# bupt-ai-cz/HIAST

Hardware: AMD Instinct MI355X
Metric: self-training images/sec (fwd+bwd+pseudo-label) at 1024x512 (higher is better)
Workload: dtype fp16

## Files before the change

### hiast_amd/csrc/conv_launch.h

```cpp
#pragma once
#include <stdlib.h>

#include "common.h"

namespace hiast {

struct IGeo {
    int H, W, Ho, Wo, stride, dil;
};

}

struct ConvLaunch {
    const void* x = nullptr;
    const void* wp = nullptr;
    void* y = nullptr;
    const void* res = nullptr;
    const void* res_gate = nullptr;
    int gate_mask = 0;
    const float* gamma = nullptr;
    const float* beta = nullptr;
    const float* mean = nullptr;
    const float* var = nullptr;
    float eps = 0.0f;
    int relu = 0;
    int64_t M = 0;
    int K = 0, N = 0, taps = 1;
    hiast::IGeo geo = {0, 0, 0, 0, 1, 1};
    int fmt = HIAST_FMT_BF16;
    int out_f32 = 0;
    float* stats = nullptr;
    int stats_rows = 0;
    int stats_mode = 0;
    hipStream_t st = nullptr;

    int planes() const { return hiast_fmt_planes(fmt); }
    bool f16() const { return fmt == HIAST_FMT_FP16; }
};

enum class ConvFamily { XCONV, XCONV2, TILE_F16, TILE };

struct ConvRoute {
    ConvFamily family = ConvFamily::TILE;
    int BN = 0, BM = 0;
    bool half9 = false;
    int rows = 0;
};

static inline int conv_panel_streams(int64_t M, int NG, int panel_rows)
{
    static const int env_cus = [] { const char* e = getenv("HIAST_XCONV_CUS"); const int v = e ? atoi(e) : 0; return v >= 8 && v <= 256 ? v : 0; }();
    const long long npanel = (M + panel_rows - 1) / panel_rows;
    long long streams = (env_cus ? env_cus : hiast_grid_cus()) / NG / 8 * 8;
    if (streams < 8) streams = 8;
    if (streams > npanel) streams = (npanel + 7) / 8 * 8;
    return (int)streams;
}

ConvRoute ig_route(const ConvLaunch& c);
int hiast_igemm_launch(const ConvLaunch& c);
int hiast_igemm_launch_f16(const ConvLaunch& c, const ConvRoute& r);
int hiast_xconv_ok(const ConvLaunch& c);
int hiast_xconv_stats_rows(int64_t M, int N);
int hiast_xconv_launch(const ConvLaunch& c, const ConvRoute& r);
int hiast_xconv2_ok(const ConvLaunch& c);
int hiast_xconv2_launch(const ConvLaunch& c);
int hiast_gemm_nt_launch(const float* x, const float* w, float* y, int64_t M, int K, int N, hipStream_t st);
```

### hiast_amd/csrc/igemm.hip

```cpp
#include "igemm_kernel.h"

namespace hiast {

template <int PL>
__device__ __forceinline__ size_t ig_wp_elem(int n, int t, int k, int taps, int KO)
{
    const size_t row = ((size_t)n * taps + t) * PL * KO;
    return PL == 2 ? row + (size_t)(k >> 5) * 64 + (k & 31) : row + k;
}

template <int PL, bool F16 = false>
__global__ __launch_bounds__(256) void pack_conv_weight_kernel(const float* __restrict__ w,
                                                               unsigned short* __restrict__ wp,
                                                               unsigned short* __restrict__ wpt, int N, int K, int taps,
                                                               int mode)
{
    const long long idx = (long long)blockIdx.x * 256 + threadIdx.x;
    if (idx >= (long long)N * taps * K) return;
    const int k = (int)(idx % K);
    const int t = (int)((idx / K) % taps);
    const int n = (int)(idx / ((long long)K * taps));
    const float v = w[((size_t)n * K + k) * taps + t];
    unsigned short h, l = 0;
    if (F16) h = H16<true>::enc(v);
    else ig_split(v, h, l);
    if (mode != 1) {
        unsigned short* d = wp + ig_wp_elem<PL>(n, t, k, taps, K);
        d[0] = h;
        if (PL == 2) d[32] = l;
    }
    if (mode != 0) {
        unsigned short* d = (mode == 1 ? wp : wpt) + ig_wp_elem<PL>(k, taps - 1 - t, n, taps, N);
        d[0] = h;
        if (PL == 2) d[32] = l;
    }
}

constexpr int PK_PITCH = 72;

template <int PL, bool F16 = false>
__device__ __forceinline__ void pack_tile(const float* __restrict__ w, unsigned short* __restrict__ wp,
                                          unsigned short* __restrict__ wpt, int N, int K, int taps, int mode, int n0,
                                          int k0, unsigned short* lds)
{
    constexpr int TN = PL == 1 ? 32 : 16;
    unsigned short* hi = lds;
    unsigned short* lo = lds + (PL == 2 ? TN * taps * PK_PITCH : 0);
    unsigned short* fwd = (mode == 1) ? nullptr : wp;
    unsigned short* adj = (mode == 0) ? nullptr : (mode == 1 ? wp : wpt);
    const int run = 64 * taps;
    for (int nh = 0; nh < 64; nh += TN) {
        if (nh) __syncthreads();
        for (int e = threadIdx.x; e < TN * run; e += 256) {
            const int n = e / run, r = e - n * run;
            const int k = r / taps, t = r - k * taps;
            const float v = w[((size_t)(n0 + nh + n) * K + k0) * taps + r];
            unsigned short h, l = 0;
            if (F16) h = H16<true>::enc(v);
            else ig_split(v, h, l);
            hi[(n * taps + t) * PK_PITCH + k] = h;
            if (PL == 2) lo[(n * taps + t) * PK_PITCH + k] = l;
        }
        __syncthreads();
        if (fwd) {
            for (int e = threadIdx.x; e < TN * taps * 8; e += 256) {
                const int c = e & 7, nt = e >> 3;
                const int n = nt / taps, t = nt - n * taps;
                const uint4 vh = *reinterpret_cast<const uint4*>(&hi[nt * PK_PITCH + c * 8]);
                unsigned short* d = fwd + ig_wp_elem<PL>(n0 + nh + n, t, k0 + c * 8, taps, K);
                *reinterpret_cast<uint4*>(d) = vh;
                if (PL == 2) *reinterpret_cast<uint4*>(d + 32) = *reinterpret_cast<const uint4*>(&lo[nt * PK_PITCH + c * 8]);
            }
        }
        if (adj) {
            for (int e = threadIdx.x; e < 64 * taps * (TN / 8); e += 256) {
                const int c = e % (TN / 8), kt = e / (TN / 8);
                const int k = kt / taps, t = kt - k * taps;
                unsigned short vh[8], vl[8];
#pragma unroll
                for (int j = 0; j < 8; ++j) {
                    vh[j] = hi[((c * 8 + j) * taps + t) * PK_PITCH + k];
                    if (PL == 2) vl[j] = lo[((c * 8 + j) * taps + t) * PK_PITCH + k];
                }
                unsigned short* d = adj + ig_wp_elem<PL>(k0 + k, taps - 1 - t, n0 + nh + c * 8, taps, N);
                *reinterpret_cast<uint4*>(d) = make_uint4(vh[0] | (unsigned)vh[1] << 16, vh[2] | (unsigned)vh[3] << 16,
                                                          vh[4] | (unsigned)vh[5] << 16, vh[6] | (unsigned)vh[7] << 16);
                if (PL == 2)
                    *reinterpret_cast<uint4*>(d + 32) = make_uint4(vl[0] | (unsigned)vl[1] << 16, vl[2] | (unsigned)vl[3] << 16,
                                                                   vl[4] | (unsigned)vl[5] << 16, vl[6] | (unsigned)vl[7] << 16);
            }
        }
    }
}

template <int PL, bool F16 = false>
__global__ __launch_bounds__(256) void pack_conv_weight_tiled_kernel(const float* __restrict__ w,
                                                                     unsigned short* __restrict__ wp,
                                                                     unsigned short* __restrict__ wpt, int N, int K,
                                                                     int taps, int mode)
{
    extern __shared__ __attribute__((aligned(16))) unsigned short lds[];
    const int kt = K / 64;
    pack_tile<PL, F16>(w, wp, wpt, N, K, taps, mode, (int)(blockIdx.x / kt) * 64, (int)(blockIdx.x % kt) * 64, lds);
}

__global__ __launch_bounds__(256) void pack_conv_weight_multi_kernel(const hiast_pack_rec* __restrict__ table,
                                                                     const int32_t* __restrict__ chunk_tensor,
                                                                     const int64_t* __restrict__ chunk_start)
{
    extern __shared__ __attribute__((aligned(16))) unsigned short lds[];
    const hiast_pack_rec r = table[chunk_tensor[blockIdx.x]];
    const int kt = r.K / 64;
    const int tile = (int)chunk_start[blockIdx.x];
    const int n0 = (tile / kt) * 64, k0 = (tile % kt) * 64;
    if (r.planes == HIAST_FMT_SPLIT_BF16)
        pack_tile<2>(r.w, (unsigned short*)r.wp, (unsigned short*)r.wpt, r.N, r.K, r.taps, r.mode, n0, k0, lds);
    else if (r.planes == HIAST_FMT_FP16)
        pack_tile<1, true>(r.w, (unsigned short*)r.wp, (unsigned short*)r.wpt, r.N, r.K, r.taps, r.mode, n0, k0, lds);
    else
        pack_tile<1>(r.w, (unsigned short*)r.wp, (unsigned short*)r.wpt, r.N, r.K, r.taps, r.mode, n0, k0, lds);
}

__global__ __launch_bounds__(256) void to_planes_kernel(const float* __restrict__ x, unsigned short* __restrict__ p,
                                                        long long M, int C)
{
    const long long total8 = M * C / 8;
    for (long long i = (long long)blockIdx.x * 256 + threadIdx.x; i < total8; i += (long long)gridDim.x * 256) {
        const long long m = (i * 8) / C;
        const int c = (int)((i * 8) - m * C);
        const float4 a = reinterpret_cast<const float4*>(x)[2 * i], b = reinterpret_cast<const float4*>(x)[2 * i + 1];
        const float v[8] = {a.x, a.y, a.z, a.w, b.x, b.y, b.z, b.w};
        unsigned ph[4], pl_[4];
#pragma unroll
        for (int q = 0; q < 4; ++q) {
            unsigned short h0, l0, h1, l1;
            ig_split(v[2 * q], h0, l0);
            ig_split(v[2 * q + 1], h1, l1);
            ph[q] = (unsigned)h0 | ((unsigned)h1 << 16);
            pl_[q] = (unsigned)l0 | ((unsigned)l1 << 16);
        }
        unsigned short* dst = p + ig_elem<2>((size_t)m, c, C);
        *reinterpret_cast<uint4*>(dst) = make_uint4(ph[0], ph[1], ph[2], ph[3]);
        *reinterpret_cast<uint4*>(dst + 32) = make_uint4(pl_[0], pl_[1], pl_[2], pl_[3]);
    }
}

__global__ __launch_bounds__(256) void from_planes_kernel(const unsigned short* __restrict__ p, float* __restrict__ x,
                                                          long long M, int C)
{
    const long long total8 = M * C / 8;
    for (long long i = (long long)blockIdx.x * 256 + threadIdx.x; i < total8; i += (long long)gridDim.x * 256) {
        const long long m = (i * 8) / C;
        const int c = (int)((i * 8) - m * C);
        const unsigned short* src = p + ig_elem<2>((size_t)m, c, C);
        const uint4 h = *reinterpret_cast<const uint4*>(src), l = *reinterpret_cast<const uint4*>(src + 32);
        const unsigned wh[4] = {h.x, h.y, h.z, h.w}, wl[4] = {l.x, l.y, l.z, l.w};
        float v[8];
#pragma unroll
        for (int q = 0; q < 4; ++q) {
            v[2 * q] = __uint_as_float(wh[q] << 16) + __uint_as_float(wl[q] << 16);
            v[2 * q + 1] = __uint_as_float(wh[q] & 0xFFFF0000u) + __uint_as_float(wl[q] & 0xFFFF0000u);
        }
        reinterpret_cast<float4*>(x)[2 * i] = make_float4(v[0], v[1], v[2], v[3]);
        reinterpret_cast<float4*>(x)[2 * i + 1] = make_float4(v[4], v[5], v[6], v[7]);
    }
}

}

struct IgEnv {
    int half;
    int bn;
    int ragged_off;
    int cosched0;
};
static const IgEnv& ig_env()
{
    static const IgEnv env = [] {
        IgEnv e;
        const char* v = getenv("HIAST_IGEMM_HALF");
        e.half = v ? (atoi(v) != 0) : -1;
        v = getenv("HIAST_IGEMM_BN");
        const int bn = v ? atoi(v) : 0;
        e.bn = (bn == 64 || bn == 128 || bn == 256) ? bn : 0;
        e.ragged_off = getenv("HIAST_IGEMM_RAGGED") != nullptr;
        v = getenv("HIAST_IGEMM_COSCHED");
        e.cosched0 = v && atoi(v) != 0;
        return e;
    }();
    return env;
}
static thread_local int ig_cosched_tls = -1, ig_half_tls = -1;
extern "C" int hiast_igemm_set_half(int v)
{
    const int prev = ig_half_tls;
    ig_half_tls = v < 0 ? -1 : (v != 0);
    return prev;
}
extern "C" int hiast_igemm_set_cosched(int on)
{
    const int prev = ig_cosched_tls;
    ig_cosched_tls = on < 0 ? -1 : (on != 0);
    return prev;
}
static int ig_half_forced() { return ig_half_tls >= 0 ? ig_half_tls : ig_env().half; }
static int ig_cosched() { return ig_cosched_tls >= 0 ? ig_cosched_tls : ig_env().cosched0; }

#ifndef IG_HALF_AUTO
#define IG_HALF_BLOCKS(M, N) ((((M) + 255) / 256) * (((N) % 256 == 0) ? (N) / 256 : (N) / 128))
#define IG_HALF_AUTO(M, K, N) (IG_HALF_BLOCKS(M, N) <= 64 || (IG_HALF_BLOCKS(M, N) <= 128 && !ig_cosched()))
#endif
static int ig_half_tile(int64_t M, int K, int N, int taps, int out_f32)
{
    if (taps != 1 || out_f32 || N % 128 != 0 || M < 4096) return 0;
    if (ig_half_forced() >= 0) return ig_half_forced();
    return IG_HALF_AUTO(M, K, N);
}
static int ig_half_tile9(int64_t M, int N, int PL, bool bn_relu_only)
{
    if (PL != 2 || !bn_relu_only || N % 128 != 0 || M < 4096) return 0;
    if (ig_half_forced() >= 0) return ig_half_forced();
    return IG_HALF_AUTO(M, 0, N);
}

ConvRoute ig_route(const ConvLaunch& c)
{
    ConvRoute r;
    if (c.stats_mode != 2 && hiast_xconv_ok(c)) {
        r.family = ConvFamily::XCONV;
        r.rows = hiast_xconv_stats_rows(c.M, c.N);
        return r;
    }
    if (c.stats_mode == 0 && !c.f16() && hiast_xconv2_ok(c)) {
        r.family = ConvFamily::XCONV2;
        return r;
    }
    r.family = c.f16() ? ConvFamily::TILE_F16 : ConvFamily::TILE;
    r.BN = (c.N % 256 == 0) ? 256 : ((c.N % 128 == 0) ? 128 : 64);
    const bool plain = !c.mean && !c.gamma && !c.res && !c.relu && !c.res_gate && c.stats_mode == 0;
    if (plain && !c.out_f32 && r.BN == 128 && c.N > 512 && !ig_env().ragged_off) r.BN = 256;
    if (const int v = ig_env().bn) {
        if (c.N % v == 0) r.BN = v;
    }
    r.half9 = c.taps == 9 && !c.out_f32 && c.geo.stride == 1 &&
              ig_half_tile9(c.M, c.N, c.planes(), c.mean && c.relu && !c.res && !c.res_gate && c.stats_mode == 0) != 0;
    const bool half = r.half9 || (c.geo.stride >= 0 && ig_half_tile(c.M, c.K, c.N, c.taps, c.out_f32) != 0);
    if (half) r.BN = 128;
    r.BM = half ? 128 : hiast::IG_BM;
    r.rows = (int)((c.M + r.BM - 1) / r.BM);
    return r;
}

int hiast_igemm_launch(const ConvLaunch& in)
{
    ConvLaunch c = in;
    if (c.stats_mode != 2) c.stats_mode = c.stats ? 1 : 0;
    const int H = c.geo.H, W = c.geo.W, stride = c.geo.stride, dil = c.geo.dil;
    if (!hiast_fmt_ok(c.fmt)) return HIAST_E_RANGE;
    const int planes = c.planes();
    if (c.stats_mode == 2) {
        if (!c.stats || !c.res || !c.mean || !c.var || planes != 1 || c.out_f32 || c.relu || c.res_gate || c.N % 8) return HIAST_E_RANGE;
    } else {
        if (c.stats && (planes != 1 || c.out_f32 || c.res || c.relu)) return HIAST_E_RANGE;
        if ((c.stats || c.res_gate) && c.mean) return HIAST_E_RANGE;
    }
    if (c.res_gate && (planes != 1 || !c.res || c.relu || c.out_f32 || (!c.gate_mask && (((uintptr_t)c.res_gate) & 15)))) return HIAST_E_RANGE;
    if (!c.x || !c.wp || !c.y || (c.mean && !c.var)) return HIAST_E_ARG;
    if (c.M <= 0 || c.K <= 0 || c.N <= 0) return HIAST_E_ARG;
    if ((planes != 1 && planes != 2) || (c.taps != 1 && c.taps != 9)) return HIAST_E_RANGE;
    if ((c.K * planes) % 64 != 0 || c.N % 64 != 0 || c.M > (1ll << 31) - 512) return HIAST_E_RANGE;
    if (c.out_f32 && c.res) return HIAST_E_RANGE;
    if ((((uintptr_t)c.x) | ((uintptr_t)c.wp) | ((uintptr_t)c.y) | ((uintptr_t)c.res)) & 15) return HIAST_E_RANGE;
    c.geo = {0, 0, 0, 0, 1, 1};
    size_t in_pix = (size_t)c.M;
    if (c.taps != 1 && stride == -2) {
        if (H <= 0 || W <= 0 || dil != 1 || planes != 1 || c.out_f32) return HIAST_E_ARG;
        const int Hs = (H - 1) / 2 + 1, Ws = (W - 1) / 2 + 1;
        if (c.M % ((int64_t)H * W) != 0) return HIAST_E_ARG;
        c.geo = {Hs, Ws, H, W, -2, 1};
        in_pix = (size_t)(c.M / ((int64_t)H * W)) * Hs * Ws;
    } else if (c.taps != 1) {
        if (H <= 0 || W <= 0 || stride <= 0 || dil <= 0) return HIAST_E_ARG;
        const int Ho = (H - 1) / stride + 1, Wo = (W - 1) / stride + 1;
        if (c.M % ((int64_t)Ho * Wo) != 0) return HIAST_E_ARG;
        c.geo = {H, W, Ho, Wo, stride, dil};
        in_pix = (size_t)(c.M / ((int64_t)Ho * Wo)) * H * W;
    }
    if (in_pix * planes * c.K * 2 >= (1ull << 31) || (size_t)c.N * c.taps * planes * c.K * 2 >= (1ull << 31)) return HIAST_E_RANGE;
    const ConvRoute r = ig_route(c);
    if (c.stats_mode != 0 && c.stats_rows != r.rows) return HIAST_E_ARG;
    switch (r.family) {
    case ConvFamily::XCONV: return hiast_xconv_launch(c, r);
    case ConvFamily::XCONV2: return hiast_xconv2_launch(c);
    case ConvFamily::TILE_F16: return hiast_igemm_launch_f16(c, r);
    case ConvFamily::TILE: break;
    }
    if (planes == 2) return c.out_f32 ? launch_igemm_t<2, true>(c, r) : launch_igemm_t<2, false>(c, r);
    return c.out_f32 ? launch_igemm_t<1, true>(c, r) : launch_igemm_t<1, false>(c, r);
}

extern "C" int hiast_igemm_dgrad_bn_stats(const void* dy, const void* wpt, void* da, int B, int H, int W, int Cin, int Cout,
                                          int taps, int dil, const void* bn_x, const float* gamma, const float* beta,
                                          const float* save_mean, const float* save_invstd, float* partial, int partial_rows,
                                          int fmt, hiast_stream_t stream)
{
    if (fmt != HIAST_FMT_BF16 && fmt != HIAST_FMT_FP16) return HIAST_E_RANGE;
    if (B <= 0 || H <= 0 || W <= 0) return HIAST_E_ARG;
    if (!bn_x || !save_mean || !save_invstd || !partial) return HIAST_E_ARG;
    if ((((uintptr_t)save_mean) | ((uintptr_t)save_invstd) | ((uintptr_t)gamma) | ((uintptr_t)beta)) & 15) return HIAST_E_RANGE;
    ConvLaunch c;
    c.x = dy; c.wp = wpt; c.y = da; c.res = bn_x;
    c.gamma = gamma; c.beta = beta; c.mean = save_mean; c.var = save_invstd;
    c.M = (int64_t)B * H * W; c.K = Cin; c.N = Cout; c.taps = taps;
    c.geo.H = H; c.geo.W = W; c.geo.dil = dil;
    c.fmt = fmt;
    c.stats = partial; c.stats_rows = partial_rows; c.stats_mode = 2;
    c.st = (hipStream_t)stream;
    return hiast_igemm_launch(c);
}

extern "C" int hiast_igemm_dgrad_s2(const void* dy, const void* wpt, void* dx, int B, int H, int W, int Cin, int Cout, int fmt,
                                    hiast_stream_t stream)
{
    if (fmt != HIAST_FMT_BF16 && fmt != HIAST_FMT_FP16) return HIAST_E_RANGE;
    if (B <= 0 || H <= 0 || W <= 0) return HIAST_E_ARG;
    ConvLaunch c;
    c.x = dy; c.wp = wpt; c.y = dx;
    c.M = (int64_t)B * H * W; c.K = Cout; c.N = Cin; c.taps = 9;
    c.geo.H = H; c.geo.W = W; c.geo.stride = -2;
    c.fmt = fmt;
    c.st = (hipStream_t)stream;
    return hiast_igemm_launch(c);
}

extern "C" int hiast_igemm_bn_act(const void* x, const void* wp, const float* gamma, const float* beta,
                                  const float* mean, const float* var, float eps, const void* res, int relu, void* y,
                                  int B, int H, int W, int Cin, int Cout, int taps, int stride, int dil, int fmt,
                                  int out_f32, float* stats, int stats_rows, const void* res_gate, int gate_mask,
                                  hiast_stream_t stream)
{
    if (B <= 0 || H <= 0 || W <= 0) return HIAST_E_ARG;
    if (taps == 1 && stride != 1) return HIAST_E_RANGE;
    const int Ho = taps == 1 ? H : (H - 1) / stride + 1, Wo = taps == 1 ? W : (W - 1) / stride + 1;
    ConvLaunch c;
    c.x = x; c.wp = wp; c.y = y; c.res = res; c.res_gate = res_gate; c.gate_mask = gate_mask;
    c.gamma = gamma; c.beta = beta; c.mean = mean; c.var = var; c.eps = eps;
    c.relu = relu;
    c.M = (int64_t)B * Ho * Wo; c.K = Cin; c.N = Cout; c.taps = taps;
    c.geo.H = H; c.geo.W = W; c.geo.stride = stride; c.geo.dil = dil;
    c.fmt = fmt; c.out_f32 = out_f32;
    c.stats = stats; c.stats_rows = stats_rows;
    c.st = (hipStream_t)stream;
    return hiast_igemm_launch(c);
}

extern "C" int hiast_igemm_stats_rows(int64_t M, int Cin, int Cout, int taps, int fmt)
{
    if (M <= 0 || Cin <= 0 || Cout <= 0) return 0;
    ConvLaunch c;
    c.M = M; c.K = Cin; c.N = Cout; c.taps = taps; c.fmt = fmt;
    c.stats_mode = 1;
    return ig_route(c).rows;
}
extern "C" int hiast_igemm_dgrad_bn_stats_rows(int64_t M, int Cin, int Cout, int taps)
{
    if (M <= 0) return 0;
    ConvLaunch c;
    c.M = M; c.K = Cin; c.N = Cout; c.taps = taps;
    c.stats_mode = 2;
    return ig_route(c).rows;
}

#ifdef IG_STAMP
namespace hiast {
__global__ void ig_stamp_copy_kernel(unsigned* dst)
{
    for (int i = blockIdx.x * blockDim.x + threadIdx.x; i < 1024 * 8 * 8 + 32 * 64; i += gridDim.x * blockDim.x) dst[i] = ig_stamp_buf[i];
}
}
extern "C" int hiast_igemm_debug_stamps(unsigned* dst_device)
{
    hipLaunchKernelGGL(hiast::ig_stamp_copy_kernel, dim3(64), dim3(256), 0, 0, dst_device);
    return (int)hipDeviceSynchronize();
}
#endif

extern "C" int hiast_pack_conv_weight(const float* w, int N, int K, int taps, int fmt, int transpose, void* wp,
                                      void* wpt, hiast_stream_t stream)
{
    if (!w || !wp) return HIAST_E_ARG;
    if (N <= 0 || K <= 0 || taps <= 0) return HIAST_E_ARG;
    const int planes = fmt;
    if (!hiast_fmt_ok(fmt) || transpose < 0 || transpose > 2) return HIAST_E_RANGE;
    if (transpose == 2 && !wpt) return HIAST_E_ARG;
    if (planes == HIAST_FMT_SPLIT_BF16 && ((transpose != 1 && K % 32 != 0) || (transpose != 0 && N % 32 != 0))) return HIAST_E_RANGE;
    const long long total = (long long)N * K * taps;
    if (N % 64 == 0 && K % 64 == 0 && taps <= 9 && !((((uintptr_t)wp) | ((uintptr_t)wpt)) & 15)) {
        const dim3 tg((unsigned)((N / 64) * (K / 64)));
        const size_t lds_bytes = (size_t)32 * taps * hiast::PK_PITCH * sizeof(unsigned short);
        if (planes == HIAST_FMT_SPLIT_BF16)
            hipLaunchKernelGGL(hiast::pack_conv_weight_tiled_kernel<2>, tg, dim3(256), lds_bytes, (hipStream_t)stream, w,
                               (unsigned short*)wp, (unsigned short*)wpt, N, K, taps, transpose);
        else if (planes == HIAST_FMT_FP16)
            hipLaunchKernelGGL((hiast::pack_conv_weight_tiled_kernel<1, true>), tg, dim3(256), lds_bytes, (hipStream_t)stream, w,
                               (unsigned short*)wp, (unsigned short*)wpt, N, K, taps, transpose);
        else
            hipLaunchKernelGGL(hiast::pack_conv_weight_tiled_kernel<1>, tg, dim3(256), lds_bytes, (hipStream_t)stream, w,
                               (unsigned short*)wp, (unsigned short*)wpt, N, K, taps, transpose);
        HIAST_CHECK_LAUNCH();
        return 0;
    }
    const dim3 grid((unsigned)((total + 255) / 256));
    if (planes == HIAST_FMT_SPLIT_BF16)
        hipLaunchKernelGGL(hiast::pack_conv_weight_kernel<2>, grid, dim3(256), 0, (hipStream_t)stream, w,
                           (unsigned short*)wp, (unsigned short*)wpt, N, K, taps, transpose);
    else if (planes == HIAST_FMT_FP16)
        hipLaunchKernelGGL((hiast::pack_conv_weight_kernel<1, true>), grid, dim3(256), 0, (hipStream_t)stream, w,
                           (unsigned short*)wp, (unsigned short*)wpt, N, K, taps, transpose);
    else
        hipLaunchKernelGGL(hiast::pack_conv_weight_kernel<1>, grid, dim3(256), 0, (hipStream_t)stream, w,
                           (unsigned short*)wp, (unsigned short*)wpt, N, K, taps, transpose);
    HIAST_CHECK_LAUNCH();
    return 0;
}

namespace hiast {

template <int INK, int PL, bool F16 = false>
__global__ __launch_bounds__(256) void stem_tail_kernel(const void* __restrict__ xv, const float* __restrict__ gamma,
                                                        const float* __restrict__ beta, const float* __restrict__ mean,
                                                        const float* __restrict__ var, float eps,
                                                        unsigned short* __restrict__ out, int B, int H, int W, int C, int Ho,
                                                        int Wo)
{
    const int G = C >> 3;
    const long long total = (long long)B * Ho * Wo * G;
    const long long stride = (long long)gridDim.x * 256;
    long long i = (long long)blockIdx.x * 256 + threadIdx.x;
    if (i >= total) return;
    const int cg = (int)(i % G);
    float sc[8], sh[8];
#pragma unroll
    for (int k = 0; k < 8; ++k) {
        const int c = cg * 8 + k;
        const float invstd = 1.0f / sqrtf(var[c] + eps);
        sc[k] = (gamma ? gamma[c] : 1.0f) * invstd;
        sh[k] = fmaf(-mean[c], sc[k], beta ? beta[c] : 0.0f);
    }
    for (; i < total; i += stride) {
        const long long pix = i / G;
        const int xo = (int)(pix % Wo);
        const int yo = (int)((pix / Wo) % Ho);
        const int b = (int)(pix / ((long long)Wo * Ho));
        float m[8];
#pragma unroll
        for (int k = 0; k < 8; ++k) m[k] = -INFINITY;
#pragma unroll
        for (int dy = 0; dy < 3; ++dy) {
            const int yy = 2 * yo - 1 + dy;
            if (yy < 0 || yy >= H) continue;
#pragma unroll
            for (int dx = 0; dx < 3; ++dx) {
                const int xx = 2 * xo - 1 + dx;
                if (xx < 0 || xx >= W) continue;
                const size_t off = (((size_t)b * H + yy) * W + xx) * C + cg * 8;
                float v[8];
                if (INK != 0) {
                    const uint4 r = *reinterpret_cast<const uint4*>(reinterpret_cast<const unsigned short*>(xv) + off);
                    const unsigned w4[4] = {r.x, r.y, r.z, r.w};
#pragma unroll
                    for (int q = 0; q < 4; ++q) {
                        v[2 * q] = H16<INK == 2>::lo(w4[q]);
                        v[2 * q + 1] = H16<INK == 2>::hi(w4[q]);
                    }
                } else {
                    const float4 a = *reinterpret_cast<const float4*>(reinterpret_cast<const float*>(xv) + off);
                    const float4 c4 = *reinterpret_cast<const float4*>(reinterpret_cast<const float*>(xv) + off + 4);
                    v[0] = a.x; v[1] = a.y; v[2] = a.z; v[3] = a.w; v[4] = c4.x; v[5] = c4.y; v[6] = c4.z; v[7] = c4.w;
                }
#pragma unroll
                for (int k = 0; k < 8; ++k) {
                    float t = fmaf(v[k], sc[k], sh[k]);
                    t = (t > 0.f || t != t) ? t : 0.f;
                    if (INK != 0) t = H16<INK == 2>::dec(H16<INK == 2>::enc(t));
                    m[k] = (t > m[k] || t != t) ? t : m[k];
                }
            }
        }
        unsigned ph[4], pl_[4];
#pragma unroll
        for (int q = 0; q < 4; ++q) {
            unsigned short h0, l0 = 0, h1, l1 = 0;
            if (PL == 2) {
                ig_split(m[2 * q], h0, l0);
                ig_split(m[2 * q + 1], h1, l1);
            } else {
                h0 = H16<F16>::enc(m[2 * q]);
                h1 = H16<F16>::enc(m[2 * q + 1]);
            }
            ph[q] = (unsigned)h0 | ((unsigned)h1 << 16);
            pl_[q] = (unsigned)l0 | ((unsigned)l1 << 16);
        }
        unsigned short* dst = out + ig_elem<PL>((size_t)pix, cg * 8, C);
        *reinterpret_cast<uint4*>(dst) = make_uint4(ph[0], ph[1], ph[2], ph[3]);
        if (PL == 2) *reinterpret_cast<uint4*>(dst + 32) = make_uint4(pl_[0], pl_[1], pl_[2], pl_[3]);
    }
}

}

extern "C" int hiast_stem_tail(const void* x, int dtype, const float* gamma, const float* beta, const float* mean,
                               const float* var, float eps, void* out, int fmt, int B, int H, int W, int C,
                               hiast_stream_t stream)
{
    if (!hiast_fmt_ok(fmt)) return HIAST_E_RANGE;
    const int planes = hiast_fmt_planes(fmt), f16 = fmt == HIAST_FMT_FP16;
    if (!x || !mean || !var || !out) return HIAST_E_ARG;
    if (B <= 0 || H <= 0 || W <= 0 || C <= 0) return HIAST_E_ARG;
    if (dtype < 0 || dtype > 2 || C % 8 != 0 || (planes == 2 && C % 32 != 0) ||
        ((((uintptr_t)x) | ((uintptr_t)out)) & 15))
        return HIAST_E_RANGE;
    const int Ho = (H - 1) / 2 + 1, Wo = (W - 1) / 2 + 1, G = C / 8;
    const long long total = (long long)B * Ho * Wo * G;
    if ((long long)B * H * W * C >= (1ll << 40)) return HIAST_E_RANGE;
    long long nb = (total + 255) / 256;
    int grid = (int)(nb > 16384 ? 16384 : nb);
    if (grid < nb) {
        long long a = 256, g = G;
        while (a) { const long long t = g % a; g = a; a = t; }
        const int need = (int)(G / g);
        if (grid >= need) grid -= grid % need;
        else return HIAST_E_RANGE;
    }
    hipStream_t st = (hipStream_t)stream;
#define L(BF, PL)                                                                                                  \
    hipLaunchKernelGGL((hiast::stem_tail_kernel<BF, PL>), dim3(grid), dim3(256), 0, st, x, gamma, beta, mean, var, eps, \
                       (unsigned short*)out, B, H, W, C, Ho, Wo)
#define LF(BF)                                                                                                     \
    hipLaunchKernelGGL((hiast::stem_tail_kernel<BF, 1, true>), dim3(grid), dim3(256), 0, st, x, gamma, beta, mean, var, eps, \
                       (unsigned short*)out, B, H, W, C, Ho, Wo)
    if (f16) { if (dtype == 2) LF(2); else if (dtype == 1) LF(1); else LF(0); }
    else if (dtype == 2) { if (planes == 2) L(2, 2); else L(2, 1); }
    else if (dtype == 1) { if (planes == 2) L(1, 2); else L(1, 1); }
    else { if (planes == 2) L(0, 2); else L(0, 1); }
#undef LF
#undef L
    HIAST_CHECK_LAUNCH();
    return 0;
}

extern "C" int hiast_split_planes(float* x, void* planes, int64_t M, int C, int inverse, hiast_stream_t stream)
{
    if (!x || !planes) return HIAST_E_ARG;
    if (M <= 0 || C <= 0) return HIAST_E_ARG;
    if (C % 32 != 0 || ((((uintptr_t)x) | ((uintptr_t)planes)) & 15)) return HIAST_E_RANGE;
    const long long total8 = (long long)M * C / 8;
    long long nb = (total8 + 255) / 256;
    const int grid = (int)(nb < 1 ? 1 : (nb > 8192 ? 8192 : nb));
    if (inverse)
        hipLaunchKernelGGL(hiast::from_planes_kernel, dim3(grid), dim3(256), 0, (hipStream_t)stream,
                           (const unsigned short*)planes, x, (long long)M, C);
    else
        hipLaunchKernelGGL(hiast::to_planes_kernel, dim3(grid), dim3(256), 0, (hipStream_t)stream, (const float*)x,
                           (unsigned short*)planes, (long long)M, C);
    HIAST_CHECK_LAUNCH();
    return 0;
}

extern "C" int hiast_pack_conv_weight_multi(const hiast_pack_rec* table, const int32_t* chunk_tensor,
                                            const int64_t* chunk_start, int n_chunks, int max_taps, hiast_stream_t stream)
{
    if (!table || !chunk_tensor || !chunk_start) return HIAST_E_ARG;
    if (n_chunks <= 0 || max_taps <= 0) return HIAST_E_ARG;
    if (max_taps > 9) return HIAST_E_RANGE;
    const size_t lds_bytes = (size_t)32 * max_taps * hiast::PK_PITCH * sizeof(unsigned short);
    hipLaunchKernelGGL(hiast::pack_conv_weight_multi_kernel, dim3(n_chunks), dim3(256), lds_bytes, (hipStream_t)stream, table,
                       chunk_tensor, chunk_start);
    HIAST_CHECK_LAUNCH();
    return 0;
}
```

### hiast_amd/csrc/xconv.hip

```cpp
#include <hip/hip_bf16.h>
#include <stdlib.h>

#include "conv_launch.h"

namespace hiast {

constexpr int XC_PANEL = 64;
constexpr int XC_STAGES = 3;
constexpr int XC_COLS = 512;

__device__ __forceinline__ h_bf16x8 xc_lds_read(unsigned addr)
{
    h_bf16x8 v;
    asm volatile("ds_read_b128 %0, %1" : "=v"(v) : "v"(addr));
    return v;
}
__device__ __forceinline__ void xc_lds_wait(h_bf16x8& a, h_bf16x8& b)
{
    asm volatile("s_waitcnt lgkmcnt(0)" : "+v"(a), "+v"(b));
}

__device__ __forceinline__ int xc_chan(int g, int b, int r) { return (b >> 1) * 32 + g * 8 + (b & 1) * 4 + r; }

template <int KC, bool BN, bool RES, bool RELU, bool GATE, bool STATS, bool F16 = false>
__global__ __launch_bounds__(512) void xconv_kernel(const unsigned short* __restrict__ X,
                                                    const unsigned short* __restrict__ Wp,
                                                    const float* __restrict__ gamma, const float* __restrict__ beta,
                                                    const float* __restrict__ mean, const float* __restrict__ var,
                                                    float eps, const unsigned short* __restrict__ R,
                                                    const unsigned char* __restrict__ Rg,
                                                    unsigned short* __restrict__ Y, int M, int N,
                                                    float* __restrict__ stats)
{
    constexpr int SL = KC / 64;
    constexpr int KS = KC / 32;
    constexpr int STAGE = XC_PANEL * KC * 2;
    __shared__ __attribute__((aligned(1024))) unsigned char smem[XC_STAGES * STAGE];
    __shared__ float s_sc[XC_COLS], s_sh[XC_COLS];

    const int tid = threadIdx.x, lane = tid & 63;
    const int wave = __builtin_amdgcn_readfirstlane(tid >> 6);
    const int g = lane >> 4, px = lane & 15;
    const int NG = N / XC_COLS;
    const int xcd = blockIdx.x & 7, slot = blockIdx.x >> 3;
    const int cg = slot % NG;
    const int nstream = (int)gridDim.x / NG;
    const int stream = (slot / NG) * 8 + xcd;
    const int n0 = cg * XC_COLS + wave * 64;
    const int npanel = (M + XC_PANEL - 1) / XC_PANEL;

    h_bf16x8 wr[4][KS];
#pragma unroll
    for (int b = 0; b < 4; ++b) {
        const unsigned short* wrow = Wp + (size_t)(n0 + xc_chan(px >> 2, b, px & 3)) * KC + g * 8;
#pragma unroll
        for (int s = 0; s < KS; ++s) wr[b][s] = *reinterpret_cast<const h_bf16x8*>(wrow + s * 32);
    }
#pragma unroll
    for (int b = 0; b < 4; ++b)
#pragma unroll
        for (int s = 0; s < KS; ++s) asm volatile("" : "+v"(wr[b][s]));
    if (BN) {
        for (int c = tid; c < XC_COLS; c += 512) {
            const int n = cg * XC_COLS + c;
            const float sc = (gamma ? gamma[n] : 1.0f) * (1.0f / sqrtf(var[n] + eps));
            s_sc[c] = sc;
            s_sh[c] = fmaf(-mean[n], sc, beta ? beta[n] : 0.0f);
        }
        __syncthreads();
    }

    constexpr int OOB = (int)0x80000000;
    const __amdgpu_buffer_rsrc_t xrs = __builtin_amdgcn_make_buffer_rsrc((void*)X, 0, (int)((size_t)M * KC * 2), 0x00020000);
    const int drow = wave * 8 + (lane >> 3);
    const int dchunk = ((lane & 7) ^ ((drow >> 1) & 7)) * 16;
    auto issue = [&](int p, int st) {
        const int m = p * XC_PANEL + drow;
        const int voff = (p < npanel && m < M) ? (int)((size_t)m * KC * 2) + dchunk : OOB;
        unsigned char* base = smem + st * STAGE + wave * 1024;
#pragma unroll
        for (int j = 0; j < SL; ++j) h_dma16(xrs, base + j * (XC_PANEL * 128), voff, j * 128);
    };

    const unsigned lds_base = (unsigned)(size_t)smem;
    float st1[STATS ? 16 : 1], st2[STATS ? 16 : 1];
#pragma unroll
    for (int q = 0; q < (STATS ? 16 : 1); ++q) { st1[q] = 0.f; st2[q] = 0.f; }

    issue(stream, 0);
    issue(stream + nstream, 1);
    int it = 0;
    for (int p = stream; p < npanel; p += nstream, ++it) {
        const int st = it % XC_STAGES;
        constexpr int NRES = RES ? (GATE ? 8 : 4) : 0;
        if (it == 0) asm volatile("s_waitcnt vmcnt(%0)\n\ts_barrier" ::"n"(SL) : "memory");
        else asm volatile("s_waitcnt vmcnt(%0)\n\ts_barrier" ::"n"(SL + 8 + NRES) : "memory");
        uint4 rres[RES ? 2 : 1][2];
        unsigned rgate[GATE ? 2 : 1][2];
        auto load_res = [&](int half) {
#pragma unroll
            for (int t = 0; t < 2; ++t) {
                const int m = p * XC_PANEL + half * 32 + t * 16 + px;
                const size_t row = (size_t)(m < M ? m : 0) * N + n0 + g * 8;
                rres[t][0] = h_load16_once(R + row);
                rres[t][1] = h_load16_once(R + row + 32);
                if (GATE) {
                    const unsigned char* gp = Rg + (size_t)(m < M ? m : 0) * (N >> 3) + ((n0 + g * 8) >> 3);
                    rgate[t][0] = gp[0];
                    rgate[t][1] = gp[4];
                }
            }
        };
        if (RES) load_res(0);
        issue(p + 2 * nstream, (it + 2) % XC_STAGES);
#pragma unroll
        for (int half = 0; half < 2; ++half) {
            if (RES && half == 1) load_res(1);
            h_f32x4 acc[2][4];
#pragma unroll
            for (int a = 0; a < 2; ++a)
#pragma unroll
                for (int b = 0; b < 4; ++b) acc[a][b] = (h_f32x4){0.f, 0.f, 0.f, 0.f};
            auto frag = [&](int s, int a) {
                return xc_lds_read(lds_base + (unsigned)(st * STAGE + (s >> 1) * (XC_PANEL * 128) +
                                                         h_lds_off(half * 32 + a * 16 + px, (s & 1) * 4 + g)));
            };
            constexpr bool DB = !(STATS || (BN && RES));
            h_bf16x8 xa[DB ? 2 : 1][2];
            xa[0][0] = frag(0, 0);
            xa[0][1] = frag(0, 1);
            xc_lds_wait(xa[0][0], xa[0][1]);
#pragma unroll
            for (int s = 0; s < KS; ++s) {
                constexpr int one = DB ? 1 : 0;
                if (DB && s + 1 < KS) {
                    xa[(s + 1) & one][0] = frag(s + 1, 0);
                    xa[(s + 1) & one][1] = frag(s + 1, 1);
                }
#pragma unroll
                for (int a = 0; a < 2; ++a)
#pragma unroll
                    for (int b = 0; b < 4; ++b)
                        acc[a][b] = H16<F16>::mfma16(wr[b][s], xa[s & one][a], acc[a][b]);
                if (s + 1 < KS) {
                    if (!DB) {
                        xa[0][0] = frag(s + 1, 0);
                        xa[0][1] = frag(s + 1, 1);
                    }
                    xc_lds_wait(xa[(s + 1) & one][0], xa[(s + 1) & one][1]);
                }
            }
#pragma unroll
            for (int a = 0; a < 2; ++a) {
                const int m = p * XC_PANEL + half * 32 + a * 16 + px;
                const bool ok = m < M;
                const size_t row = (size_t)(ok ? m : 0) * N + n0 + g * 8;
                const uint4 r0 = rres[RES ? a : 0][0], r1 = rres[RES ? a : 0][1];
                const unsigned gate0 = GATE ? rgate[GATE ? a : 0][0] : 0xFFu;
                const unsigned gate1 = GATE ? rgate[GATE ? a : 0][1] : 0xFFu;
                float o[16];
#pragma unroll
                for (int b = 0; b < 4; ++b)
#pragma unroll
                    for (int r = 0; r < 4; ++r) o[(b >> 1) * 8 + (b & 1) * 4 + r] = acc[a][b][r];
                if (BN) {
#pragma unroll
                    for (int hh = 0; hh < 2; ++hh) {
                        const int c = wave * 64 + hh * 32 + g * 8;
#pragma unroll
                        for (int q = 0; q < 8; q += 4) {
                            const float4 sc = *reinterpret_cast<const float4*>(&s_sc[c + q]);
                            const float4 sh = *reinterpret_cast<const float4*>(&s_sh[c + q]);
                            o[hh * 8 + q] = fmaf(o[hh * 8 + q], sc.x, sh.x);
                            o[hh * 8 + q + 1] = fmaf(o[hh * 8 + q + 1], sc.y, sh.y);
                            o[hh * 8 + q + 2] = fmaf(o[hh * 8 + q + 2], sc.z, sh.z);
                            o[hh * 8 + q + 3] = fmaf(o[hh * 8 + q + 3], sc.w, sh.w);
                        }
                    }
                }
                if (RES) {
                    const unsigned w0[4] = {r0.x, r0.y, r0.z, r0.w}, w1[4] = {r1.x, r1.y, r1.z, r1.w};
#pragma unroll
                    for (int q = 0; q < 4; ++q) {
                        float a0 = H16<F16>::lo(w0[q]), a1 = H16<F16>::hi(w0[q]);
                        float b0 = H16<F16>::lo(w1[q]), b1 = H16<F16>::hi(w1[q]);
                        if (GATE) {
                            a0 = ((gate0 >> (2 * q)) & 1u) ? a0 : 0.f;
                            a1 = ((gate0 >> (2 * q + 1)) & 1u) ? a1 : 0.f;
                            b0 = ((gate1 >> (2 * q)) & 1u) ? b0 : 0.f;
                            b1 = ((gate1 >> (2 * q + 1)) & 1u) ? b1 : 0.f;
                        }
                        o[2 * q] += a0;
                        o[2 * q + 1] += a1;
                        o[8 + 2 * q] += b0;
                        o[8 + 2 * q + 1] += b1;
                    }
                }
                if (RELU) {
#pragma unroll
                    for (int q = 0; q < 16; ++q) o[q] = o[q] > 0.f ? o[q] : 0.f;
                }
                unsigned pk[8];
                if (STATS && F16) {
#pragma unroll
                    for (int q = 0; q < 8; ++q) {
                        pk[q] = H16<F16>::pack(o[2 * q], o[2 * q + 1]);
                        if (ok) {
                            const float v0 = H16<F16>::lo(pk[q]), v1 = H16<F16>::hi(pk[q]);
                            st1[2 * q] += v0; st2[2 * q] = fmaf(v0, v0, st2[2 * q]);
                            st1[2 * q + 1] += v1; st2[2 * q + 1] = fmaf(v1, v1, st2[2 * q + 1]);
                        }
                        __builtin_amdgcn_sched_barrier(0);
                    }
                } else {
#pragma unroll
                    for (int q = 0; q < 8; ++q) pk[q] = H16<F16>::pack(o[2 * q], o[2 * q + 1]);
                    if (STATS && ok) {
#pragma unroll
                        for (int q = 0; q < 8; ++q) {
                            const float v0 = H16<F16>::lo(pk[q]), v1 = H16<F16>::hi(pk[q]);
                            st1[2 * q] += v0; st2[2 * q] = fmaf(v0, v0, st2[2 * q]);
                            st1[2 * q + 1] += v1; st2[2 * q + 1] = fmaf(v1, v1, st2[2 * q + 1]);
                        }
                    }
                }
                if (ok) {
                    h_store16_out(Y + row, pk[0], pk[1], pk[2], pk[3]);
                    h_store16_out(Y + row + 32, pk[4], pk[5], pk[6], pk[7]);
                }
            }
        }
    }
    if (STATS) {
#pragma unroll
        for (int q = 0; q < 16; ++q) {
#pragma unroll
            for (int o = 1; o < 16; o <<= 1) {
                st1[q] += __shfl_xor(st1[q], o, 64);
                st2[q] += __shfl_xor(st2[q], o, 64);
            }
        }
        if (px == 0) {
            float* d = stats + ((size_t)stream * N + n0 + g * 8) * 2;
#pragma unroll
            for (int q = 0; q < 8; ++q) {
                d[2 * q] = st1[q];
                d[2 * q + 1] = st2[q];
                d[64 + 2 * q] = st1[8 + q];
                d[64 + 2 * q + 1] = st2[8 + q];
            }
        }
    }
}

}

int hiast_xconv_ok(const ConvLaunch& c)
{
    const char* env = getenv("HIAST_XCONV");
    const bool has_bn = c.mean != nullptr, has_res = c.res != nullptr;
    if ((env && atoi(env) == 0) || c.planes() != 1 || c.taps != 1 || c.out_f32) return 0;
    if (c.K != 256 || c.N % hiast::XC_COLS != 0 || c.N > 2048) return 0;
    if (c.res_gate && (!c.gate_mask || !has_res || c.relu)) return 0;
    if (has_bn && has_res && !c.relu) return 0;
    if (c.stats_mode == 1 && (has_res || c.relu || has_bn)) return 0;
    if (c.M < 4096) return 0;
    return 1;
}

int hiast_xconv_stats_rows(int64_t M, int N)
{
    return conv_panel_streams(M, N / hiast::XC_COLS, hiast::XC_PANEL);
}

int hiast_xconv_launch(const ConvLaunch& c, const ConvRoute& r)
{
    using namespace hiast;
    const dim3 grid((unsigned)(r.rows * (c.N / XC_COLS)));
#define XK(BNF, RESF, RELUF, GATEF, STATSF, F16)                                                                      \
    hipLaunchKernelGGL((xconv_kernel<256, BNF, RESF, RELUF, GATEF, STATSF, F16>), grid, dim3(512), 0, c.st,           \
                       (const unsigned short*)c.x, (const unsigned short*)c.wp, c.gamma, c.beta, c.mean, c.var, c.eps, \
                       (const unsigned short*)c.res, (const unsigned char*)c.res_gate, (unsigned short*)c.y, (int)c.M, c.N, \
                       c.stats)
#define XL(BNF, RESF, RELUF, GATEF, STATSF)                                                                          \
    do {                                                                                                             \
        if (c.f16()) XK(BNF, RESF, RELUF, GATEF, STATSF, true);                                                      \
        else XK(BNF, RESF, RELUF, GATEF, STATSF, false);                                                             \
    } while (0)
    const bool bn = c.mean != nullptr;
    if (c.stats) { XL(false, false, false, false, true); }
    else if (c.res_gate) { XL(false, true, false, true, false); }
    else if (c.res) {
        if (bn) { if (c.relu) XL(true, true, true, false, false); else return HIAST_E_RANGE; }
        else { if (c.relu) XL(false, true, true, false, false); else XL(false, true, false, false, false); }
    } else {
        if (bn) { if (c.relu) XL(true, false, true, false, false); else XL(true, false, false, false, false); }
        else { if (c.relu) XL(false, false, true, false, false); else XL(false, false, false, false, false); }
    }
#undef XL
#undef XK
    HIAST_CHECK_LAUNCH();
    return 0;
}
```

Baseline: 144.0.

## Add weight-stationary K=512 1x1 conv kernel and route eligible convs to it

Adds a new xconv512 kernel for 1x1 convolutions with K=512 and N a multiple of 256 (N>=1024). Each wave keeps its weight slice in registers while streaming 32-row activation panels through a 3-stage LDS pipeline via buffer DMA, with fused BN/residual/gate/ReLU/stats epilogues. The router now sends these shapes to the new kernel instead of the generic tiled igemm. The risk is high register pressure from holding 32 weight vectors per lane, which lowers occupancy, and stats row counts now depend on the chosen form.

```diff
diff --git a/hiast_amd/csrc/conv_launch.h b/hiast_amd/csrc/conv_launch.h
--- a/hiast_amd/csrc/conv_launch.h
+++ b/hiast_amd/csrc/conv_launch.h
@@ -38,7 +38,7 @@
     bool f16() const { return fmt == HIAST_FMT_FP16; }
 };
 
-enum class ConvFamily { XCONV, XCONV2, TILE_F16, TILE };
+enum class ConvFamily { XCONV, XCONV512, XCONV2, TILE_F16, TILE };
 
 struct ConvRoute {
     ConvFamily family = ConvFamily::TILE;
@@ -61,8 +61,10 @@
 int hiast_igemm_launch(const ConvLaunch& c);
 int hiast_igemm_launch_f16(const ConvLaunch& c, const ConvRoute& r);
 int hiast_xconv_ok(const ConvLaunch& c);
-int hiast_xconv_stats_rows(int64_t M, int N);
+int hiast_xconv_stats_rows(int64_t M, int N, int form);
 int hiast_xconv_launch(const ConvLaunch& c, const ConvRoute& r);
+int hiast_xconv512_stats_rows(int64_t M, int N);
+int hiast_xconv512_launch(const ConvLaunch& c, const ConvRoute& r);
 int hiast_xconv2_ok(const ConvLaunch& c);
 int hiast_xconv2_launch(const ConvLaunch& c);
 int hiast_gemm_nt_launch(const float* x, const float* w, float* y, int64_t M, int K, int N, hipStream_t st);
diff --git a/hiast_amd/csrc/igemm.hip b/hiast_amd/csrc/igemm.hip
--- a/hiast_amd/csrc/igemm.hip
+++ b/hiast_amd/csrc/igemm.hip
@@ -226,9 +226,9 @@
 ConvRoute ig_route(const ConvLaunch& c)
 {
     ConvRoute r;
-    if (c.stats_mode != 2 && hiast_xconv_ok(c)) {
-        r.family = ConvFamily::XCONV;
-        r.rows = hiast_xconv_stats_rows(c.M, c.N);
+    if (const int form = c.stats_mode != 2 ? hiast_xconv_ok(c) : 0) {
+        r.family = form == 512 ? ConvFamily::XCONV512 : ConvFamily::XCONV;
+        r.rows = hiast_xconv_stats_rows(c.M, c.N, form);
         return r;
     }
     if (c.stats_mode == 0 && !c.f16() && hiast_xconv2_ok(c)) {
@@ -291,6 +291,7 @@
     if (c.stats_mode != 0 && c.stats_rows != r.rows) return HIAST_E_ARG;
     switch (r.family) {
     case ConvFamily::XCONV: return hiast_xconv_launch(c, r);
+    case ConvFamily::XCONV512: return hiast_xconv512_launch(c, r);
     case ConvFamily::XCONV2: return hiast_xconv2_launch(c);
     case ConvFamily::TILE_F16: return hiast_igemm_launch_f16(c, r);
     case ConvFamily::TILE: break;
diff --git a/hiast_amd/csrc/xconv.hip b/hiast_amd/csrc/xconv.hip
--- a/hiast_amd/csrc/xconv.hip
+++ b/hiast_amd/csrc/xconv.hip
@@ -260,16 +260,24 @@
     const char* env = getenv("HIAST_XCONV");
     const bool has_bn = c.mean != nullptr, has_res = c.res != nullptr;
     if ((env && atoi(env) == 0) || c.planes() != 1 || c.taps != 1 || c.out_f32) return 0;
-    if (c.K != 256 || c.N % hiast::XC_COLS != 0 || c.N > 2048) return 0;
     if (c.res_gate && (!c.gate_mask || !has_res || c.relu)) return 0;
     if (has_bn && has_res && !c.relu) return 0;
     if (c.stats_mode == 1 && (has_res || c.relu || has_bn)) return 0;
     if (c.M < 4096) return 0;
-    return 1;
-}
-
-int hiast_xconv_stats_rows(int64_t M, int N)
-{
+    if (c.K == 256) return (c.N % hiast::XC_COLS == 0 && c.N <= 2048) ? 256 : 0;
+    if (c.K == 512) {
+        const char* env5 = getenv("HIAST_XCONV_K512");
+        if ((env5 && atoi(env5) == 0) || c.N % 256 != 0 || c.N < 1024) return 0;
+        if (c.relu && !has_bn && !has_res) return 0;
+        if (has_res && c.N < 2048) return 0;
+        return 512;
+    }
+    return 0;
+}
+
+int hiast_xconv_stats_rows(int64_t M, int N, int form)
+{
+    if (form == 512) return hiast_xconv512_stats_rows(M, N);
     return conv_panel_streams(M, N / hiast::XC_COLS, hiast::XC_PANEL);
 }
 
diff --git a/hiast_amd/csrc/xconv512.hip b/hiast_amd/csrc/xconv512.hip
--- /dev/null
+++ b/hiast_amd/csrc/xconv512.hip
@@ -0,0 +1,269 @@
+#include <hip/hip_bf16.h>
+#include <stdlib.h>
+
+#include "conv_launch.h"
+
+namespace hiast {
+
+constexpr int X5_PANEL = 32;
+constexpr int X5_STAGES = 3;
+constexpr int X5_COLS = 256;
+constexpr int X5_KC = 512;
+
+template <int IDX>
+__device__ __forceinline__ h_bf16x8 x5_lds_read_i(unsigned addr)
+{
+    h_bf16x8 v;
+    asm volatile("ds_read_b128 %0, %1 offset:%2" : "=v"(v) : "v"(addr), "i"(IDX * 2048));
+    return v;
+}
+__device__ __forceinline__ h_bf16x8 x5_lds_read(unsigned addr, int idx)
+{
+    switch (idx) {
+    case 1: return x5_lds_read_i<1>(addr);
+    case 2: return x5_lds_read_i<2>(addr);
+    case 3: return x5_lds_read_i<3>(addr);
+    case 4: return x5_lds_read_i<4>(addr);
+    case 5: return x5_lds_read_i<5>(addr);
+    case 6: return x5_lds_read_i<6>(addr);
+    case 7: return x5_lds_read_i<7>(addr);
+    case 8: return x5_lds_read_i<8>(addr);
+    case 9: return x5_lds_read_i<9>(addr);
+    case 10: return x5_lds_read_i<10>(addr);
+    case 11: return x5_lds_read_i<11>(addr);
+    case 12: return x5_lds_read_i<12>(addr);
+    case 13: return x5_lds_read_i<13>(addr);
+    case 14: return x5_lds_read_i<14>(addr);
+    case 15: return x5_lds_read_i<15>(addr);
+    default: return x5_lds_read_i<0>(addr);
+    }
+}
+__device__ __forceinline__ void x5_lds_wait(h_bf16x8& a, h_bf16x8& b, h_bf16x8& c, h_bf16x8& d)
+{
+    asm volatile("s_waitcnt lgkmcnt(0)" : "+v"(a), "+v"(b), "+v"(c), "+v"(d));
+}
+
+template <bool BN, bool RES, bool RELU, bool GATE, bool STATS, bool F16>
+__global__ __launch_bounds__(512) void xconv512_kernel(const unsigned short* __restrict__ X, const unsigned short* __restrict__ Wp,
+                                                       const float* __restrict__ gamma, const float* __restrict__ beta,
+                                                       const float* __restrict__ mean, const float* __restrict__ var, float eps,
+                                                       const unsigned short* __restrict__ R, const unsigned char* __restrict__ Rg,
+                                                       unsigned short* __restrict__ Y, int M, int N, float* __restrict__ stats)
+{
+    constexpr int SL = X5_KC / 64;
+    constexpr int KS = X5_KC / 32;
+    constexpr int STAGE = X5_PANEL * X5_KC * 2;
+    constexpr int NDMA = SL * (X5_PANEL / 8) / 8;
+    __shared__ __attribute__((aligned(1024))) unsigned char smem[X5_STAGES * STAGE];
+
+    const int tid = threadIdx.x, lane = tid & 63;
+    const int wave = __builtin_amdgcn_readfirstlane(tid >> 6);
+    const int g = lane >> 4, px = lane & 15;
+    const int NG = N / X5_COLS;
+    const int xcd = blockIdx.x & 7, slot = blockIdx.x >> 3;
+    const int cg = slot % NG;
+    const int nstream = (int)gridDim.x / NG;
+    const int stream = (slot / NG) * 8 + xcd;
+    const int n0 = cg * X5_COLS + wave * 32;
+    const int npanel = (M + X5_PANEL - 1) / X5_PANEL;
+    const int c0 = n0 + g * 8;
+
+    h_bf16x8 wr[2][KS];
+#pragma unroll
+    for (int b = 0; b < 2; ++b) {
+        const unsigned short* wrow = Wp + (size_t)(n0 + (px >> 2) * 8 + b * 4 + (px & 3)) * X5_KC + g * 8;
+#pragma unroll
+        for (int s = 0; s < KS; ++s) wr[b][s] = *reinterpret_cast<const h_bf16x8*>(wrow + s * 32);
+    }
+#pragma unroll
+    for (int b = 0; b < 2; ++b)
+#pragma unroll
+        for (int s = 0; s < KS; ++s) asm volatile("" : "+v"(wr[b][s]));
+    float sc[BN ? 8 : 1], sh[BN ? 8 : 1];
+    if (BN) {
+#pragma unroll
+        for (int q = 0; q < 8; ++q) {
+            const int n = c0 + q;
+            sc[q] = (gamma ? gamma[n] : 1.0f) * (1.0f / sqrtf(var[n] + eps));
+            sh[q] = fmaf(-mean[n], sc[q], beta ? beta[n] : 0.0f);
+        }
+#pragma unroll
+        for (int q = 0; q < 8; ++q) asm volatile("" : "+v"(sc[q]), "+v"(sh[q]));
+    }
+
+    constexpr int OOB = (int)0x80000000;
+    const __amdgpu_buffer_rsrc_t xrs = __builtin_amdgcn_make_buffer_rsrc((void*)X, 0, (int)((size_t)M * X5_KC * 2), 0x00020000);
+    const int drow = (wave & 3) * 8 + (lane >> 3);
+    const int dslab = (wave >> 2) * NDMA;
+    const int dchunk = dslab * 128 + ((lane & 7) ^ ((drow >> 1) & 7)) * 16;
+    auto issue = [&](int p, int st) {
+        const int m = p * X5_PANEL + drow;
+        const int voff = (p < npanel && m < M) ? (int)((size_t)m * X5_KC * 2) + dchunk : OOB;
+        unsigned char* base = smem + st * STAGE + dslab * (X5_PANEL * 128) + (wave & 3) * 1024;
+#pragma unroll
+        for (int j = 0; j < NDMA; ++j) h_dma16(xrs, base + j * (X5_PANEL * 128), voff, j * 128);
+    };
+    const unsigned lds_base = (unsigned)(size_t)smem;
+    float st1[STATS ? 8 : 1], st2[STATS ? 8 : 1];
+#pragma unroll
+    for (int q = 0; q < (STATS ? 8 : 1); ++q) { st1[q] = 0.f; st2[q] = 0.f; }
+
+    constexpr int NROW = RES ? (GATE ? 4 : 2) : 0;
+    struct Rows {
+        uint4 res[2];
+        unsigned gate[2];
+    };
+    Rows ring[2];
+    auto load_rows = [&](Rows& r, int p) {
+        if (!RES) return;
+#pragma unroll
+        for (int t = 0; t < 2; ++t) {
+            const int m = p * X5_PANEL + t * 16 + px;
+            const size_t mr = (size_t)((p < npanel && m < M) ? m : 0);
+            r.res[t] = h_load16_once(R + mr * N + c0);
+            if (GATE) r.gate[t] = Rg[mr * (N >> 3) + (c0 >> 3)];
+        }
+    };
+    auto panel = [&](int p, int it, const Rows& cur, Rows& nxt) {
+        const int st = it % X5_STAGES;
+        if (it == 0) asm volatile("s_waitcnt vmcnt(%0)\n\ts_barrier" ::"n"(NDMA) : "memory");
+        else asm volatile("s_waitcnt vmcnt(%0)\n\ts_barrier" ::"n"(NDMA + 2 + NROW) : "memory");
+        load_rows(nxt, p + nstream);
+        issue(p + 2 * nstream, (it + 2) % X5_STAGES);
+        const unsigned fbase = lds_base + (unsigned)(st * STAGE) + (unsigned)h_lds_off(px, g);
+        h_f32x4 acc[2][2];
+#pragma unroll
+        for (int a = 0; a < 2; ++a)
+#pragma unroll
+            for (int b = 0; b < 2; ++b) acc[a][b] = (h_f32x4){0.f, 0.f, 0.f, 0.f};
+        h_bf16x8 xa[2][2][2];
+        auto request = [&](int j) {
+#pragma unroll
+            for (int o = 0; o < 2; ++o)
+#pragma unroll
+                for (int a = 0; a < 2; ++a) xa[j & 1][o][a] = x5_lds_read(o ? fbase ^ 64u : fbase, 2 * j + a);
+        };
+        auto landed = [&](int j) { x5_lds_wait(xa[j & 1][0][0], xa[j & 1][0][1], xa[j & 1][1][0], xa[j & 1][1][1]); };
+        request(0);
+        landed(0);
+#pragma unroll
+        for (int j = 0; j < SL; ++j) {
+            if (j + 1 < SL) request(j + 1);
+#pragma unroll
+            for (int o = 0; o < 2; ++o)
+#pragma unroll
+                for (int a = 0; a < 2; ++a)
+#pragma unroll
+                    for (int b = 0; b < 2; ++b) acc[a][b] = H16<F16>::mfma16(wr[b][2 * j + o], xa[j & 1][o][a], acc[a][b]);
+            if (j + 1 < SL) landed(j + 1);
+        }
+#pragma unroll
+        for (int a = 0; a < 2; ++a) {
+            const int m = p * X5_PANEL + a * 16 + px;
+            const bool ok = m < M;
+            float o[8];
+#pragma unroll
+            for (int b = 0; b < 2; ++b)
+#pragma unroll
+                for (int r = 0; r < 4; ++r) o[b * 4 + r] = acc[a][b][r];
+            if (BN) {
+#pragma unroll
+                for (int q = 0; q < 8; ++q) o[q] = fmaf(o[q], sc[BN ? q : 0], sh[BN ? q : 0]);
+            }
+            if (RES) {
+                const unsigned w0[4] = {cur.res[a].x, cur.res[a].y, cur.res[a].z, cur.res[a].w};
+                const unsigned gate = GATE ? cur.gate[a] : 0xFFu;
+#pragma unroll
+                for (int q = 0; q < 4; ++q) {
+                    float a0 = H16<F16>::lo(w0[q]), a1 = H16<F16>::hi(w0[q]);
+                    if (GATE) {
+                        a0 = ((gate >> (2 * q)) & 1u) ? a0 : 0.f;
+                        a1 = ((gate >> (2 * q + 1)) & 1u) ? a1 : 0.f;
+                    }
+                    o[2 * q] += a0;
+                    o[2 * q + 1] += a1;
+                }
+            }
+            if (RELU) {
+#pragma unroll
+                for (int q = 0; q < 8; ++q) o[q] = o[q] > 0.f ? o[q] : 0.f;
+            }
+            unsigned pk[4];
+#pragma unroll
+            for (int q = 0; q < 4; ++q) pk[q] = H16<F16>::pack(o[2 * q], o[2 * q + 1]);
+            if (STATS && ok) {
+#pragma unroll
+                for (int q = 0; q < 4; ++q) {
+                    const float v0 = H16<F16>::lo(pk[q]), v1 = H16<F16>::hi(pk[q]);
+                    st1[2 * q] += v0; st2[2 * q] = fmaf(v0, v0, st2[2 * q]);
+                    st1[2 * q + 1] += v1; st2[2 * q + 1] = fmaf(v1, v1, st2[2 * q + 1]);
+                }
+            }
+            if (ok) h_store16_out(Y + (size_t)m * N + c0, pk[0], pk[1], pk[2], pk[3]);
+        }
+    };
+
+    load_rows(ring[0], stream);
+    issue(stream, 0);
+    issue(stream + nstream, 1);
+    for (int p = stream, it = 0; p < npanel; p += 2 * nstream, it += 2) {
+        panel(p, it, ring[0], ring[1]);
+        if (p + nstream >= npanel) break;
+        panel(p + nstream, it + 1, ring[1], ring[0]);
+    }
+    if (STATS) {
+#pragma unroll
+        for (int q = 0; q < 8; ++q) {
+#pragma unroll
+            for (int o = 1; o < 16; o <<= 1) {
+                st1[q] += __shfl_xor(st1[q], o, 64);
+                st2[q] += __shfl_xor(st2[q], o, 64);
+            }
+        }
+        if (px == 0) {
+            float* d = stats + ((size_t)stream * N + c0) * 2;
+#pragma unroll
+            for (int q = 0; q < 8; ++q) {
+                d[2 * q] = st1[q];
+                d[2 * q + 1] = st2[q];
+            }
+        }
+    }
+}
+
+}
+
+int hiast_xconv512_stats_rows(int64_t M, int N)
+{
+    return conv_panel_streams(M, N / hiast::X5_COLS, hiast::X5_PANEL);
+}
+
+int hiast_xconv512_launch(const ConvLaunch& c, const ConvRoute& r)
+{
+    using namespace hiast;
+    const dim3 grid((unsigned)(r.rows * (c.N / X5_COLS)));
+#define XK(BNF, RESF, RELUF, GATEF, STATSF, F16)                                                                      \
+    hipLaunchKernelGGL((xconv512_kernel<BNF, RESF, RELUF, GATEF, STATSF, F16>), grid, dim3(512), 0, c.st,             \
+                       (const unsigned short*)c.x, (const unsigned short*)c.wp, c.gamma, c.beta, c.mean, c.var, c.eps, \
+                       (const unsigned short*)c.res, (const unsigned char*)c.res_gate, (unsigned short*)c.y, (int)c.M, c.N, \
+                       c.stats)
+#define XL(BNF, RESF, RELUF, GATEF, STATSF)                                                                          \
+    do {                                                                                                             \
+        if (c.f16()) XK(BNF, RESF, RELUF, GATEF, STATSF, true);                                                      \
+        else XK(BNF, RESF, RELUF, GATEF, STATSF, false);                                                             \
+    } while (0)
+    const bool bn = c.mean != nullptr;
+    if (c.stats) { XL(false, false, false, false, true); }
+    else if (c.res_gate) { XL(false, true, false, true, false); }
+    else if (c.res) {
+        if (bn) { if (c.relu) XL(true, true, true, false, false); else return HIAST_E_RANGE; }
+        else { if (c.relu) XL(false, true, true, false, false); else XL(false, true, false, false, false); }
+    } else {
+        if (bn) { if (c.relu) XL(true, false, true, false, false); else XL(true, false, false, false, false); }
+        else { if (c.relu) return HIAST_E_RANGE; else XL(false, false, false, false, false); }
+    }
+#undef XL
+#undef XK
+    HIAST_CHECK_LAUNCH();
+    return 0;
+}
```

Result: slower. 139.8 (-2.9%).
